# ishine/tts-max

Measured on AMD Instinct MI355X. Metric: audio-codes/sec + RTF@24kHz, TTS-1 bs=1/32, at 1/2/4/8 MI355X, higher is better.
Workload: dtype bf16; 1 GPU; tts1 bf16 bs=1/GPU: prompt 202 tokens (150 codes), 500 greedy codes, codec codec-24k on 650 codes; model=TTS-1 (Llama-3.2-1B dims, V=193856, tied) + xcodec2-style codec codec-24k, global_batch=1, seq_len=702, parallelism=dp1

## Files before the change

### tts-max_amd/csrc/lm_attn_core.h

```cpp
#pragma once
#include "hip_common.h"

namespace tts {

template <int D, int PW>
struct DecShape {
  static constexpr int MT = PW / 16;
  static constexpr int KS = D / 32;
  static constexpr int PS = PW / 32;
  static constexpr int DT = D / 16;
};

constexpr int DEC_G = 4;
constexpr int DEC_NW = 16;
template <int D> constexpr int dec_nw() { return 16; }
template <int D> constexpr int dec_pw() { return D == 64 ? 64 : 32; }

TTS_DEV int vt_off(int S, int d, int p) {
  return (((d >> 4) * (S >> 5) + (p >> 5)) * 16 + (d & 15)) * 32 + (p & 31);
}

TTS_DEV int dec_pos(int base, int mt, int row) {
  return base + 32 * (mt >> 1) + 8 * (row >> 2) + 4 * (mt & 1) + (row & 3);
}

template <int D, int PW, bool O32 = false>
TTS_DEV void dec_load_k(const bf16_t* kc, int base, int ctx, int lane,
                        u32x4_t (&kf)[DecShape<D, PW>::MT][DecShape<D, PW>::KS]) {
  using C = DecShape<D, PW>;
  const int c = lane & 15, g = lane >> 4;
#pragma unroll
  for (int mt = 0; mt < C::MT; ++mt) {
    const int p = min(dec_pos(base, mt, c), ctx - 1);
#pragma unroll
    for (int ks = 0; ks < C::KS; ++ks)
      kf[mt][ks] = O32 ? *(const u32x4_t*)(kc + (p * D + 32 * ks + 8 * g))
                       : *(const u32x4_t*)(kc + (size_t)p * D + 32 * ks + 8 * g);
  }
}
template <int D, int PW, bool O32 = false>
TTS_DEV void dec_load_v(const bf16_t* vtc, int S, int base, int lane,
                        u32x4_t (&vf)[DecShape<D, PW>::PS][DecShape<D, PW>::DT]) {
  using C = DecShape<D, PW>;
  const int c = lane & 15, g = lane >> 4;
#pragma unroll
  for (int ps = 0; ps < C::PS; ++ps) {
    const int pb = min((base >> 5) + ps, (S >> 5) - 1);
    const int o0 = (pb * 16 + c) * 32 + 8 * g;
#pragma unroll
    for (int dt = 0; dt < C::DT; ++dt)
      vf[ps][dt] = O32 ? *(const u32x4_t*)(vtc + (o0 + dt * 16 * S)) : *(const u32x4_t*)(vtc + o0 + (size_t)dt * 16 * S);
  }
}

TTS_DEV uint32_t bits_sel(uint32_t mask, uint32_t a, uint32_t b) { return (a & mask) | (b & ~mask); }
template <int PW>
TTS_DEV bool dec_tail(int base, int ctx) { return __builtin_amdgcn_readfirstlane(base + PW > ctx - 1) != 0; }
template <int D, int PW>
TTS_DEV void dec_patch_k(int base, int ctx, int lane, const bf16_t* knew,
                         u32x4_t (&kf)[DecShape<D, PW>::MT][DecShape<D, PW>::KS]) {
  using C = DecShape<D, PW>;
  const int c = lane & 15, g = lane >> 4, pn = ctx - 1;
  uint32_t m[C::MT];
#pragma unroll
  for (int mt = 0; mt < C::MT; ++mt) m[mt] = dec_pos(base, mt, c) == pn ? 0xffffffffu : 0u;
#pragma unroll
  for (int ks = 0; ks < C::KS; ++ks) {
    const u32x4_t kn = *(const u32x4_t*)(knew + 32 * ks + 8 * g);
#pragma unroll
    for (int mt = 0; mt < C::MT; ++mt)
#pragma unroll
      for (int q = 0; q < 4; ++q) kf[mt][ks][q] = bits_sel(m[mt], kn[q], kf[mt][ks][q]);
  }
}
template <int D, int PW>
TTS_DEV void dec_patch_v(int base, int ctx, int lane, const bf16_t* vnew,
                         u32x4_t (&vf)[DecShape<D, PW>::PS][DecShape<D, PW>::DT]) {
  using C = DecShape<D, PW>;
  const int c = lane & 15, g = lane >> 4, pn = ctx - 1;
  uint32_t vn[C::DT];
#pragma unroll
  for (int dt = 0; dt < C::DT; ++dt) vn[dt] = vnew[16 * dt + c];
#pragma unroll
  for (int ps = 0; ps < C::PS; ++ps) {
    const int p0 = base + 32 * ps + 8 * g;
    uint32_t keep[4], put[4];
#pragma unroll
    for (int e2 = 0; e2 < 4; ++e2) {
      const int pl = p0 + 2 * e2, ph = pl + 1;
      keep[e2] = (pl < pn ? 0x0000ffffu : 0u) | (ph < pn ? 0xffff0000u : 0u);
      put[e2] = (pl == pn ? 0x0000ffffu : 0u) | (ph == pn ? 0xffff0000u : 0u);
    }
#pragma unroll
    for (int dt = 0; dt < C::DT; ++dt) {
      const uint32_t nv = vn[dt] | (vn[dt] << 16);
#pragma unroll
      for (int e2 = 0; e2 < 4; ++e2) vf[ps][dt][e2] = (vf[ps][dt][e2] & keep[e2]) | (nv & put[e2]);
    }
  }
}

template <int D>
TTS_DEV bf16x8_t dec_qfrag(const bf16_t* qs, int lane, int ks) {
  const int h = (lane & 15) & 3, g = lane >> 4;
  return __builtin_bit_cast(bf16x8_t, *(const u32x4_t*)(qs + h * D + 32 * ks + 8 * g));
}

template <int D, int PW>
TTS_DEV void dec_scores(const u32x4_t (&kf)[DecShape<D, PW>::MT][DecShape<D, PW>::KS], const bf16_t* qs,
                        int base, int ctx, float scale, int lane, bool tail, f32x4_t (&s)[DecShape<D, PW>::MT]) {
  using C = DecShape<D, PW>;
  const int g = lane >> 4;
#pragma unroll
  for (int mt = 0; mt < C::MT; ++mt) s[mt] = f32x4_t{0.f, 0.f, 0.f, 0.f};
#pragma unroll
  for (int ks = 0; ks < C::KS; ++ks) {
    const bf16x8_t qb = dec_qfrag<D>(qs, lane, ks);
#pragma unroll
    for (int mt = 0; mt < C::MT; ++mt)
      s[mt] = __builtin_amdgcn_mfma_f32_16x16x32_bf16(__builtin_bit_cast(bf16x8_t, kf[mt][ks]), qb, s[mt], 0, 0, 0);
  }
#pragma unroll
  for (int mt = 0; mt < C::MT; ++mt)
#pragma unroll
    for (int r = 0; r < 4; ++r) s[mt][r] *= scale;
  __builtin_amdgcn_sched_barrier(0);
  if (tail) {
#pragma unroll
    for (int mt = 0; mt < C::MT; ++mt)
#pragma unroll
      for (int r = 0; r < 4; ++r) s[mt][r] = (dec_pos(base, mt, 4 * g + r) < ctx) ? s[mt][r] : -INFINITY;
    __builtin_amdgcn_sched_barrier(0);
  }
  __builtin_amdgcn_sched_barrier(0);
}

template <int D, int PW>
TTS_DEV void dec_pv(float M, float& lsum, f32x4_t (&s)[DecShape<D, PW>::MT],
                    const u32x4_t (&vf)[DecShape<D, PW>::PS][DecShape<D, PW>::DT], f32x4_t (&o)[DecShape<D, PW>::DT]) {
  using C = DecShape<D, PW>;
#pragma unroll
  for (int mt = 0; mt < C::MT; ++mt)
#pragma unroll
    for (int r = 0; r < 4; ++r) {
      const float p = __builtin_amdgcn_exp2f((s[mt][r] - M) * 1.44269504088896341f);
      lsum += p;
      s[mt][r] = p;
    }
#pragma unroll
  for (int ps = 0; ps < C::PS; ++ps) {
    const u32x4_t pw = {pack_bf2(s[2 * ps][0], s[2 * ps][1]), pack_bf2(s[2 * ps][2], s[2 * ps][3]),
                        pack_bf2(s[2 * ps + 1][0], s[2 * ps + 1][1]), pack_bf2(s[2 * ps + 1][2], s[2 * ps + 1][3])};
    const bf16x8_t pb = __builtin_bit_cast(bf16x8_t, pw);
#pragma unroll
    for (int dt = 0; dt < C::DT; ++dt)
      o[dt] = __builtin_amdgcn_mfma_f32_16x16x32_bf16(__builtin_bit_cast(bf16x8_t, vf[ps][dt]), pb, o[dt], 0, 0, 0);
  }
}

template <int D, int NW>
constexpr int dec_red_floats() { return NW * DEC_G * 2 + NW * DEC_G * D; }

template <int D, int PW, int NW, class Bar, bool O32 = false>
TTS_DEV void dec_attend_w(const bf16_t* kc, const bf16_t* vtc, int S, int ctx, float scale, const bf16_t* qs,
                          const bf16_t* knew, const bf16_t* vnew, float* red,
                          u32x4_t (&kf0)[DecShape<D, PW>::MT][DecShape<D, PW>::KS],
                          u32x4_t (&vf0)[DecShape<D, PW>::PS][DecShape<D, PW>::DT], bf16_t* out, int wave,
                          int tid, Bar bar, unsigned long long* stp = nullptr, uint64_t* gout = nullptr,
                          uint32_t gtag = 0) {
  using C = DecShape<D, PW>;
  const int lane = tid & 63;
  const int c = lane & 15, g = lane >> 4;
  const int npass = (ctx + NW * PW - 1) / (NW * PW);
  float* mred = red;
  float* lred = red + NW * DEC_G;
  float* ored = lred + NW * DEC_G;
  const int base0 = wave * PW;

  f32x4_t s0[C::MT];
  float mx = -INFINITY;
  const bool tail0 = dec_tail<PW>(base0, ctx);
  if (base0 < ctx) {
    __builtin_amdgcn_sched_barrier(0);
    if (tail0) {
      dec_patch_k<D, PW>(base0, ctx, lane, knew, kf0);
      __builtin_amdgcn_sched_barrier(0);
    }
    __builtin_amdgcn_sched_barrier(0);
    dec_scores<D, PW>(kf0, qs, base0, ctx, scale, lane, tail0, s0);
#pragma unroll
    for (int mt = 0; mt < C::MT; ++mt)
#pragma unroll
      for (int r = 0; r < 4; ++r) mx = fmaxf(mx, s0[mt][r]);
  }
  for (int ps = 1; ps < npass; ++ps) {
    const int base = (ps * NW + wave) * PW;
    if (base >= ctx) break;
    u32x4_t kf[C::MT][C::KS];
    dec_load_k<D, PW, O32>(kc, base, ctx, lane, kf);
    const bool tail = dec_tail<PW>(base, ctx);
    __builtin_amdgcn_sched_barrier(0);
    if (tail) {
      dec_patch_k<D, PW>(base, ctx, lane, knew, kf);
      __builtin_amdgcn_sched_barrier(0);
    }
    __builtin_amdgcn_sched_barrier(0);
    f32x4_t s[C::MT];
    dec_scores<D, PW>(kf, qs, base, ctx, scale, lane, tail, s);
#pragma unroll
    for (int mt = 0; mt < C::MT; ++mt)
#pragma unroll
      for (int r = 0; r < 4; ++r) mx = fmaxf(mx, s[mt][r]);
  }
  mx = fmaxf(mx, __shfl_xor(mx, 16, 64));
  mx = fmaxf(mx, __shfl_xor(mx, 32, 64));
  if (lane < DEC_G) mred[wave * DEC_G + lane] = mx;
  __builtin_amdgcn_sched_barrier(0);
  if (base0 < ctx && tail0) {
    dec_patch_v<D, PW>(base0, ctx, lane, vnew, vf0);
    __builtin_amdgcn_sched_barrier(0);
  }
  __builtin_amdgcn_sched_barrier(0);
  bar();
  TTS_STAMP(stp, 5);
  float M = -INFINITY;
#pragma unroll
  for (int w = 0; w < NW; ++w) M = fmaxf(M, mred[w * DEC_G + (c & 3)]);

  float lsum = 0.f;
  f32x4_t o[C::DT];
#pragma unroll
  for (int dt = 0; dt < C::DT; ++dt) o[dt] = f32x4_t{0.f, 0.f, 0.f, 0.f};
  if (base0 < ctx) dec_pv<D, PW>(M, lsum, s0, vf0, o);
  for (int ps = 1; ps < npass; ++ps) {
    const int base = (ps * NW + wave) * PW;
    if (base >= ctx) break;
    u32x4_t kf[C::MT][C::KS], vf[C::PS][C::DT];
    dec_load_v<D, PW, O32>(vtc, S, base, lane, vf);
    dec_load_k<D, PW, O32>(kc, base, ctx, lane, kf);
    const bool tail = dec_tail<PW>(base, ctx);
    __builtin_amdgcn_sched_barrier(0);
    if (tail) {
      dec_patch_k<D, PW>(base, ctx, lane, knew, kf);
      __builtin_amdgcn_sched_barrier(0);
    }
    __builtin_amdgcn_sched_barrier(0);
    f32x4_t s[C::MT];
    dec_scores<D, PW>(kf, qs, base, ctx, scale, lane, tail, s);
    if (tail) {
      dec_patch_v<D, PW>(base, ctx, lane, vnew, vf);
      __builtin_amdgcn_sched_barrier(0);
    }
    __builtin_amdgcn_sched_barrier(0);
    dec_pv<D, PW>(M, lsum, s, vf, o);
  }
  lsum += __shfl_xor(lsum, 16, 64);
  lsum += __shfl_xor(lsum, 32, 64);
  if (c < DEC_G) {
#pragma unroll
    for (int dt = 0; dt < C::DT; ++dt)
      *(float4*)(ored + (wave * DEC_G + c) * D + 16 * dt + 4 * g) = make_float4(o[dt][0], o[dt][1], o[dt][2], o[dt][3]);
    if (g == 0) lred[wave * DEC_G + c] = lsum;
  }
  bar();
  TTS_STAMP(stp, 6);
  static_assert(DEC_G * D <= NW * 64, "one output element per thread");
  bf16_t gob = 0;
  for (int i = tid; i < DEC_G * D; i += NW * 64) {
    const int h = i / D, d = i - h * D;
    float v[NW];
#pragma unroll
    for (int w = 0; w < NW; ++w) v[w] = lred[w * DEC_G + h];
    float O = 0.f, L = 0.f;
#pragma unroll
    for (int w = 0; w < NW; ++w) L += v[w];
#pragma unroll
    for (int w = 0; w < NW; ++w) v[w] = ored[(w * DEC_G + h) * D + d];
#pragma unroll
    for (int w = 0; w < NW; ++w) O += v[w];
    const bf16_t ob = f2bf(O / L);
    out[h * D + d] = ob;
    if (gout) gob = ob;
  }
  if (gout) {
    const uint32_t nb = (uint32_t)__builtin_amdgcn_update_dpp(0, (int)gob, 0xB1, 0xf, 0xf, false);
    if (tid < DEC_G * D && !(tid & 1))
      __hip_atomic_store(gout + (tid >> 1), ((uint64_t)gtag << 32) | (nb << 16) | gob, __ATOMIC_RELAXED,
                         __HIP_MEMORY_SCOPE_AGENT);
  }
}

template <int D, int PW, int NW, bool O32 = false>
TTS_DEV void dec_attend(const bf16_t* kc, const bf16_t* vtc, int S, int ctx, float scale, const bf16_t* qs,
                        const bf16_t* knew, const bf16_t* vnew, float* red,
                        u32x4_t (&kf0)[DecShape<D, PW>::MT][DecShape<D, PW>::KS],
                        u32x4_t (&vf0)[DecShape<D, PW>::PS][DecShape<D, PW>::DT], bf16_t* out,
                        unsigned long long* stp = nullptr, uint64_t* gout = nullptr, uint32_t gtag = 0) {
  auto bar = [] { lds_barrier(); };
  dec_attend_w<D, PW, NW, decltype(bar), O32>(kc, vtc, S, ctx, scale, qs, knew, vnew, red, kf0, vf0, out,
                          __builtin_amdgcn_readfirstlane(threadIdx.x >> 6), threadIdx.x, bar, stp, gout, gtag);
}

TTS_DEV float rope_elem(bf16_t x, bf16_t xr, bool lower_half, float c, float sn) {
  const float rot = lower_half ? -bf2f(xr) : bf2f(xr);
  return rbf(rbf(bf2f(x) * c) + rbf(rot * sn));
}

}
```

### tts-max_amd/csrc/lm_gemm_kernel.h

```cpp
#pragma once
#include <algorithm>
#include <cstdio>
#include <stdexcept>
#include <type_traits>

#include "hip_common.h"
#include "lm_kernels.h"
#include "lm_attn_core.h"

namespace tts {

constexpr int wgemm_ea(int waves) { return waves >= 16 ? 1 : (waves >= 8 ? 2 : 4); }
__host__ __device__ inline int wgemm_red_floats(int waves, int ksplit, int ng, int mt, int M, int Kl) {
  const int upw = waves / ksplit;
  int r = upw * (ksplit - 1) * ng * mt * 4 * 64;
  r = r > upw * mt * 16 * 2 ? r : upw * mt * 16 * 2;
  const int segs = (M * (Kl / 8) + 63) / 64;
  r = r > segs ? r : segs;
  r = r > Kl / 2 ? r : Kl / 2;
  return r + 64;
}

constexpr int wgemm_fattn_d(int ku) { return ku == 2 ? 64 : 128; }
template <int D>
constexpr size_t fattn_lds_bytes() {
  return (size_t)(DEC_G * D + 2 * D) * 2 + (size_t)dec_red_floats<D, DEC_NW>() * 4;
}
template <typename Poll>
TTS_DEV bool fattn_wait(Poll ready, int* err, int spins, bool report) {
  for (int n = 1; !ready(); ++n) {
    if (n > spins) {
      if (report) __hip_atomic_store(err, 1, __ATOMIC_RELAXED, __HIP_MEMORY_SCOPE_AGENT);
      return false;
    }
    if ((n & 511) == 0 && __hip_atomic_load(err, __ATOMIC_RELAXED, __HIP_MEMORY_SCOPE_AGENT)) return false;
    __builtin_amdgcn_s_sleep(1);
  }
  return true;
}

template <int NT, int D>
TTS_DEV void fattn_consumer(const WgemmArgs& wa, char* smem, int b) {
  static_assert(NT == DEC_NW * 64, "the fused attention runs on 16-wave workgroups");
  constexpr int PW = dec_pw<D>(), G = DEC_G, H2 = D / 2;
  using C = DecShape<D, PW>;
  const AttnArgs& a = wa.fa;
  bf16_t* qs = (bf16_t*)smem;
  bf16_t* knew = qs + G * D;
  bf16_t* vnew = knew + D;
  float* red = (float*)(vnew + D);
  const int tid = threadIdx.x, lane = tid & 63;
  const int wave = __builtin_amdgcn_readfirstlane(tid >> 6);
  const int row = b / a.KVH, kvh = b % a.KVH;
  const int slot = a.row_slot[row], pos = a.row_pos[row], ctx = pos + 1;
  const size_t kvbase = ((size_t)slot * a.KVH + kvh) * a.max_seq * D;
  const bf16_t* kc = a.kcache + kvbase;
  const bf16_t* vtc = a.vtcache + kvbase;
  unsigned long long* stp = wa.stamps ? wa.stamps + (size_t)blockIdx.x * 32 : nullptr;
  TTS_STAMP(stp, 0);
  u32x4_t kf[C::MT][C::KS], vf[C::PS][C::DT];
  if (wave * PW < ctx) {
    dec_load_k<D, PW, D == 128>(kc, wave * PW, ctx, lane, kf);
    dec_load_v<D, PW, D == 128>(vtc, a.max_seq, wave * PW, lane, vf);
  }
  const int qd = (2 * tid) % D;
  const uint32_t cs2 = *(const uint32_t*)(a.rope_cos + (size_t)pos * D + qd);
  const uint32_t sn2 = *(const uint32_t*)(a.rope_sin + (size_t)pos * D + qd);

  const uint32_t tag = ((uint32_t)pos << 6) | (uint32_t)wa.fattn_layer;
  const int nq = G * D / 2, ngr = nq + D;
  uint32_t raw = 0;
  if (tid < ngr) {
    int col;
    if (tid < nq) col = kvh * G * D + 2 * tid;
    else if (tid < nq + D / 2) col = a.H * D + kvh * D + 2 * (tid - nq);
    else col = a.H * D + a.KVH * D + kvh * D + 2 * (tid - nq - D / 2);
    const uint64_t* gp = wa.gran + (size_t)row * (a.ld_qkv / 2) + col / 2;
    uint64_t v;
    fattn_wait([&] {
      v = __hip_atomic_load(gp, __ATOMIC_RELAXED, __HIP_MEMORY_SCOPE_AGENT);
      return (uint32_t)(v >> 32) == tag;
    }, wa.fattn_err, wa.fattn_spins, true);
    raw = (uint32_t)v;
  }
#ifdef TTS_STAMPS
  lds_barrier();
#endif
  TTS_STAMP(stp, 1);
  const uint32_t rawr = (uint32_t)__shfl_xor((int)raw, D / 4, 64);
  if (tid < ngr) {
    uint32_t w = raw;
    if (tid < nq + D / 2) {
      const bool lower = qd < H2;
      w = pack_bf2(rope_elem((bf16_t)raw, (bf16_t)rawr, lower, bf_lo(cs2), bf_lo(sn2)),
                   rope_elem((bf16_t)(raw >> 16), (bf16_t)(rawr >> 16), lower, bf_hi(cs2), bf_hi(sn2)));
    }
    ((uint32_t*)qs)[tid] = w;
  }
  lds_barrier();
  TTS_STAMP(stp, 2);
  dec_attend<D, PW, DEC_NW, D == 128>(kc, vtc, a.max_seq, ctx, a.scale, qs, knew, vnew, red, kf, vf,
                            a.out + (size_t)row * a.H * D + kvh * G * D, stp,
                            wa.fo_units ? wa.gran + (size_t)wa.M * (wa.N / 2) + (size_t)row * (a.H * D / 2) + kvh * G * D / 2
                                        : nullptr,
                            tag);
  TTS_STAMP(stp, 3);
  if (tid < D) {
    a.kcache[kvbase + (size_t)pos * D + tid] = knew[tid];
    a.vtcache[kvbase + vt_off(a.max_seq, tid, pos)] = vnew[tid];
  }
}

TTS_DEV bf16x8_t as_bf16x8(u32x4_t v) { return __builtin_bit_cast(bf16x8_t, v); }

template <int KU, int KSPLIT, int R>
TTS_DEV void fused_oproj(const WgemmArgs& a, bf16_t* xs, float* red, int wave, int lane, uint32_t tag, int u) {
  const int kpart = wave % KSPLIT;
  const int nr = min(a.fo_ur, a.fo_units);
  u32x4_t wr[R][KU];
#pragma unroll
  for (int st = 0; st < R; ++st)
#pragma unroll
    for (int kk = 0; kk < KU; ++kk)
      wr[st][kk] = __builtin_nontemporal_load((const u32x4_t*)a.fo_w +
                                              ((((long long)st * nr + u) * KSPLIT + kpart) * KU + kk) * 64 + lane);
  const bf16_t rr = a.fo_resid[u * 16 + (lane & 15)];
  const uint64_t* g = a.gran + a.N / 2 + kpart * 64 + lane;
  uint64_t v;
  fattn_wait([&] {
    v = __hip_atomic_load(g, __ATOMIC_RELAXED, __HIP_MEMORY_SCOPE_AGENT);
    return (bool)__all((uint32_t)(v >> 32) == tag);
  }, a.fattn_err, a.fattn_spins, lane == 0);
  *(uint32_t*)(xs + kpart * 128 + 2 * lane) = (uint32_t)v;
  asm volatile("s_waitcnt lgkmcnt(0)" ::: "memory");
  f32x4_t acc = {0.f, 0.f, 0.f, 0.f};
  const int akoff = 8 * (lane >> 4);
#pragma unroll
  for (int st = 0; st < R; ++st)
#pragma unroll
    for (int kk = 0; kk < KU; ++kk) {
      const int k = ((kpart * R + st) * KU + kk) * 32 + akoff;
      const u32x4_t av = *(const u32x4_t*)(xs + k);
      acc = __builtin_amdgcn_mfma_f32_16x16x32_bf16(as_bf16x8(av), as_bf16x8(wr[st][kk]), acc, 0, 0, 0);
    }
  if (kpart > 0) *(f32x4_t*)(red + ((size_t)(kpart - 1) * 64 + lane) * 4) = acc;
  lds_barrier();
  if (kpart == 0) {
    constexpr int HB = 8;
#pragma unroll
    for (int p0 = 1; p0 < KSPLIT; p0 += HB) {
      f32x4_t pv[HB];
#pragma unroll
      for (int j = 0; j < HB; ++j)
        if (p0 + j < KSPLIT) pv[j] = *(const f32x4_t*)(red + ((size_t)(p0 + j - 1) * 64 + lane) * 4);
#pragma unroll
      for (int j = 0; j < HB; ++j)
        if (p0 + j < KSPLIT) acc += pv[j];
    }
    if (lane < 16) a.fo_resid[u * 16 + lane] = f2bf(bf2f(rr) + rbf(acc[0]));
  }
}

template <int KU, int KSPLIT, int R>
TTS_DEV void fused_oproj_rows(const WgemmArgs& a, bf16_t* xs, float* red, int wave, int lane, int u) {
  const int M = a.M, HD = a.fa.H * a.fa.D, ldxs = HD + 8, hid = a.fo_units * 16;
  unsigned long long* stp = a.stamps ? a.stamps + (size_t)blockIdx.x * 32 : nullptr;
  TTS_STAMP(stp, 0);
  const int kpart = wave % KSPLIT;
  const int nr = min(a.fo_ur, a.fo_units);
  const int KTc = (HD >> 5) / a.fo_kc, kt_pc = KTc / KSPLIT, Sc = kt_pc / KU;
  auto ktile = [&](int st, int kk) {
    const int ch = st / Sc;
    return ch * KTc + kpart * kt_pc + (st - ch * Sc) * KU + kk;
  };
  u32x4_t wr[R][KU];
#pragma unroll
  for (int st = 0; st < R; ++st)
#pragma unroll
    for (int kk = 0; kk < KU; ++kk)
      wr[st][kk] = __builtin_nontemporal_load((const u32x4_t*)a.fo_w +
                                              ((((long long)st * nr + u) * KSPLIT + kpart) * KU + kk) * 64 + lane);
  bf16_t rr[4];
#pragma unroll
  for (int r = 0; r < 4; ++r) rr[r] = a.fo_resid[(size_t)min(4 * (lane >> 4) + r, M - 1) * hid + u * 16 + (lane & 15)];
  constexpr int NGL = R * KU >= 4 ? R * KU / 4 : 1;
  int col[NGL];
#pragma unroll
  for (int j = 0; j < NGL; ++j) {
    const int gi = j * 64 + lane, ktl = gi >> 4;
    col[j] = ktile(ktl / KU, ktl % KU) * 32 + (gi & 15) * 2;
  }
  const uint64_t* g0 = a.gran + (size_t)M * (a.N / 2);
  constexpr int RB = NGL >= 4 ? 1 : 4;
  for (int m0 = 0; m0 < M; m0 += RB) {
    uint32_t tag[RB];
#pragma unroll
    for (int rb = 0; rb < RB; ++rb)
      tag[rb] = ((uint32_t)a.fa.row_pos[min(m0 + rb, M - 1)] << 6) | (uint32_t)a.fattn_layer;
    uint64_t v[RB][NGL];
    fattn_wait([&] {
      bool ok = true;
#pragma unroll
      for (int rb = 0; rb < RB; ++rb)
#pragma unroll
        for (int j = 0; j < NGL; ++j) {
          v[rb][j] = __hip_atomic_load(g0 + (size_t)min(m0 + rb, M - 1) * (HD / 2) + col[j] / 2, __ATOMIC_RELAXED,
                                       __HIP_MEMORY_SCOPE_AGENT);
          ok = ok && (uint32_t)(v[rb][j] >> 32) == tag[rb];
        }
      return (bool)__all(ok);
    }, a.fattn_err, a.fattn_spins, lane == 0);
#pragma unroll
    for (int rb = 0; rb < RB; ++rb)
      if (m0 + rb < M) {
#pragma unroll
        for (int j = 0; j < NGL; ++j) *(uint32_t*)(xs + (size_t)(m0 + rb) * ldxs + col[j]) = (uint32_t)v[rb][j];
      }
    if (m0 == 0) TTS_STAMP(stp, 1);
  }
  TTS_STAMP(stp, 2);
  asm volatile("s_waitcnt lgkmcnt(0)" ::: "memory");
  f32x4_t acc = {0.f, 0.f, 0.f, 0.f};
  const bf16_t* xr = xs + (size_t)min(lane & 15, M - 1) * ldxs + 8 * (lane >> 4);
#pragma unroll
  for (int st = 0; st < R; ++st)
#pragma unroll
    for (int kk = 0; kk < KU; ++kk) {
      const u32x4_t av = *(const u32x4_t*)(xr + ktile(st, kk) * 32);
      acc = __builtin_amdgcn_mfma_f32_16x16x32_bf16(as_bf16x8(av), as_bf16x8(wr[st][kk]), acc, 0, 0, 0);
    }
  if (kpart > 0) *(f32x4_t*)(red + ((size_t)(kpart - 1) * 64 + lane) * 4) = acc;
  lds_barrier();
  if (kpart == 0) {
    constexpr int HB = 8;
#pragma unroll
    for (int p0 = 1; p0 < KSPLIT; p0 += HB) {
      f32x4_t pv[HB];
#pragma unroll
      for (int j = 0; j < HB; ++j)
        if (p0 + j < KSPLIT) pv[j] = *(const f32x4_t*)(red + ((size_t)(p0 + j - 1) * 64 + lane) * 4);
#pragma unroll
      for (int j = 0; j < HB; ++j)
        if (p0 + j < KSPLIT) acc += pv[j];
    }
#pragma unroll
    for (int r = 0; r < 4; ++r) {
      const int m = 4 * (lane >> 4) + r;
      if (m < M) a.fo_resid[(size_t)m * hid + u * 16 + (lane & 15)] = f2bf(bf2f(rr[r]) + rbf(acc[r]));
    }
  }
  TTS_STAMP(stp, 3);
}


TTS_DEV void argmax_merge(float& v, int& i, float v2, int i2) {
  if (v2 > v || (v2 == v && i2 < i)) { v = v2; i = i2; }
}

constexpr int A_GLOBAL = 0, A_LDS = 1;

template <int WAVES, int KU, int MT_MAX, int NG, int KSPLIT, int ASRC, bool NORM, int EPI, int R,
          bool EARLY, int KSW = KSPLIT, bool FROWS = false>
__global__ __launch_bounds__(WAVES * 64) void wgemm_kernel(WgemmArgs a) {
  extern __shared__ __attribute__((aligned(16))) char smem[];
  constexpr int NT = WAVES * 64;
  constexpr bool FATT = EPI == EPI_STORE && ASRC == A_LDS && WAVES == DEC_NW && KSW == KSPLIT && MT_MAX == 1 &&
                        ((EARLY && !FROWS && wgemm_fattn_d(KU) == 64) || (!EARLY && FROWS));
  const int fo_wgs = (FATT && a.fattn_wgs) ? a.fo_units : 0;
  const int nproj = (int)gridDim.x - (FATT ? a.fattn_wgs : 0) - fo_wgs;
  if constexpr (FATT) {
    if (a.fattn_wgs) {
      const int cb = (int)blockIdx.x - nproj;
      if (cb >= 0 && cb < a.fattn_wgs) {
        fattn_consumer<NT, wgemm_fattn_d(KU)>(a, smem, cb);
        return;
      }
      if (cb >= a.fattn_wgs) {
        const int lane = threadIdx.x & 63;
        const int wave = __builtin_amdgcn_readfirstlane(threadIdx.x >> 6);
        const size_t xs_bytes = (((size_t)a.M * (a.K + 8) * 2 + 15) & ~(size_t)15);
        if constexpr (FROWS) {
          fused_oproj_rows<KU, KSPLIT, R>(a, (bf16_t*)smem, (float*)(smem + xs_bytes), wave, lane, cb - a.fattn_wgs);
        } else {
          const uint32_t tag = ((uint32_t)a.fa.row_pos[0] << 6) | (uint32_t)a.fattn_layer;
          fused_oproj<KU, KSPLIT, R>(a, (bf16_t*)smem, (float*)(smem + xs_bytes), wave, lane, tag, cb - a.fattn_wgs);
        }
        return;
      }
    }
  }
  constexpr int UPW = WAVES / KSW;
  constexpr int SL = KSPLIT / KSW;
  const int bx = (int)blockIdx.x;
  unsigned long long* stp = a.stamps ? a.stamps + (size_t)blockIdx.x * 32 : nullptr;
  TTS_STAMP(stp, 0);
  const int lane = threadIdx.x & 63;
  const int wave = __builtin_amdgcn_readfirstlane(threadIdx.x >> 6);
  const int kq = wave % KSW;
  const int kpart = (SL > 1 ? (int)blockIdx.y * KSW : 0) + kq;
  const int ugrp = wave / KSW;
  const int M = a.M;
  const int mtn = (M + 15) >> 4;
  const int cs2 = a.csplit == 2 ? 1 : 0;
  const int bunits = (a.N >> 4) / NG;
  const int units = bunits << cs2;
  const int kc = a.kc;
  const int KT = a.sliced ? (a.K >> 5) * kc : (a.K >> 5) * SL;
  const int KTc = KT / kc;
  const int kt_pc = KTc / KSPLIT;
  const int Sc = kt_pc / KU;
  const int st_off = a.sliced ? blockIdx.y * Sc : 0;
  const int kt_base = a.sliced ? blockIdx.y * KTc : (SL > 1 ? (int)blockIdx.y * (a.K >> 5) : 0);
  const bf16_t* xg = a.x ? a.x + ((a.sliced || SL > 1) ? (size_t)blockIdx.y * a.K : 0) : nullptr;
  const int ldxs = a.K + 8;
  const int ustride = nproj * UPW;

  bf16_t* xs = (bf16_t*)smem;
  const size_t xs_bytes = (ASRC != A_GLOBAL) ? (((size_t)M * ldxs * 2 + 15) & ~(size_t)15) : 0;
  float* red = (float*)(smem + xs_bytes);

  const int ur = a.ur;
  auto stile = [&](int uu, int st) -> long long {
    uu = min(uu, units - 1) >> cs2;
    const int r = uu / ur, ui = uu - r * ur;
    const int nr = min(ur, bunits - r * ur);
    return (long long)r * ur * KT * NG + (((long long)(st + st_off) * nr + ui) * KSPLIT + kpart) * NG * KU;
  };
  const int S = a.sliced ? Sc : kc * Sc;

  const int tid = threadIdx.x;
  const int kch = a.K >> 3;
  constexpr bool FTAGS = FATT && !EARLY;
  int ftag_pos = 0;
  if constexpr (FTAGS) {
    if (a.fattn_wgs) ftag_pos = a.fa.row_pos[min(lane & 15, M - 1)];
  }
  constexpr int EA = wgemm_ea(WAVES);
  const int achunks = M * kch;
  const int a_nj = (achunks + NT - 1) / NT;
  constexpr bool early_a = EARLY && ASRC == A_LDS;
  u32x4_t xe[EA], ne[EA];
  if constexpr (early_a) {
    {
#pragma unroll
      for (int j = 0; j < EA; ++j) {
        const int c = min(tid + j * NT, achunks - 1);
        const int m = c / kch, k = (c - m * kch) * 8;
        xe[j] = *(const u32x4_t*)(xg + (size_t)m * a.ldx + k);
        if constexpr (NORM) ne[j] = *(const u32x4_t*)(a.normw + k);
      }
    }
  }
  constexpr bool glds_ok = ASRC == A_LDS && !early_a;
  constexpr bool use_glds = glds_ok;
  if constexpr (glds_ok) {
    if (use_glds) {
      const int ppr = a.K >> 9;
      const int pieces = M * ppr;
      for (int p = wave; p < pieces; p += WAVES) {
        const int m = p / ppr, kp = p - m * ppr;
        __builtin_amdgcn_global_load_lds((gptr_t)(xg + (size_t)m * a.ldx + kp * 512 + lane * 8),
                                         (lptr_t)(xs + (size_t)m * ldxs + kp * 512), 16, 0, 0);
      }
      if constexpr (NORM) {
        for (int p = wave; p < ppr; p += WAVES)
          __builtin_amdgcn_global_load_lds((gptr_t)(a.normw + p * 512 + lane * 8), (lptr_t)((bf16_t*)red + p * 512),
                                           16, 0, 0);
      }
    }
  }
  int u = bx * UPW + ugrp;
  const int u_first = min(u, units - 1);
  bf16_t rre[MT_MAX][4];
  int eosr[MT_MAX][4];
  uint32_t seen_cur[MT_MAX][4];
#pragma unroll
  for (int mt = 0; mt < MT_MAX; ++mt)
#pragma unroll
    for (int r = 0; r < 4; ++r) {
      const int m = min(mt * 16 + 4 * (lane >> 4) + r, M - 1);
      if constexpr (EPI == EPI_RESID) {
        rre[mt][r] = a.resid[(size_t)m * a.ldo + (u_first >> cs2) * 16 + (lane & 15)];
      }
      if constexpr (EPI == EPI_LOGITS) {
        eosr[mt][r] = a.eos_mask[m];
        seen_cur[mt][r] = a.seen[(size_t)m * a.seen_stride + (u_first >> 1)];
      }
    }

  uint32_t ftag = 0;
  if constexpr (FATT && EARLY) {
    if (a.fattn_wgs) ftag = ((uint32_t)a.fa.row_pos[0] << 6) | (uint32_t)a.fattn_layer;
  }

  const uint32_t wbytes = (uint32_t)((long long)(a.N >> 4) * KT * 1024);
  const __amdgpu_buffer_rsrc_t wrsrc = __builtin_amdgcn_make_buffer_rsrc((void*)a.w, (short)0, (int)wbytes, 0x00020000);
  constexpr uint32_t kPast = kWgemmSentinel - (uint32_t)(NG * KU - 1) * 1024u;
  auto soff = [&](int uu, int st) -> uint32_t {
    const int ls = cs2 ? ((lane & ~8) | ((min(uu, units - 1) & 1) << 3)) : lane;
    return uu < units ? (uint32_t)stile(uu, st) * 1024u + (uint32_t)ls * 16u : kPast;
  };
  u32x4_t wr[R][KU][NG];
  constexpr bool AGR = ASRC == A_GLOBAL && MT_MAX <= 2;
  const int arow = lane & 15;
  const int akoff = 8 * (lane >> 4);
  u32x4_t ar[R][KU][AGR ? MT_MAX : 1];
  int pu = u, ps = 0;
  auto issue = [&](u32x4_t (&dst)[KU][NG], u32x4_t (&adst)[KU][AGR ? MT_MAX : 1]) {
    const uint32_t q = soff(pu, ps);
#pragma unroll
    for (int kk = 0; kk < KU; ++kk)
#pragma unroll
      for (int g = 0; g < NG; ++g)
        dst[kk][g] = __builtin_amdgcn_raw_buffer_load_b128(wrsrc, (int)(q + (uint32_t)((g * KU + kk) * 1024)), 0, 2);
    if constexpr (AGR) {
      const int sg = ps + st_off, ch = kc == 1 ? 0 : sg / Sc;
      const int kt = ch * KTc + kpart * kt_pc + (sg - ch * Sc) * KU - kt_base;
#pragma unroll
      for (int kk = 0; kk < KU; ++kk)
#pragma unroll
        for (int mt = 0; mt < MT_MAX; ++mt) {
          const int m = min(mt * 16 + arow, M - 1);
          adst[kk][mt] = *(const u32x4_t*)(xg + (size_t)m * a.ldx + (kt + kk) * 32 + akoff);
        }
    }
    if (++ps == S) { ps = 0; pu += ustride; }
  };
  __builtin_amdgcn_sched_barrier(0);
  if (a.diag & kWgemmDiagMask & 8) __syncthreads();
#pragma unroll
  for (int j = 0; j < R; ++j) issue(wr[j], ar[j]);
  __builtin_amdgcn_sched_barrier(0);

  if (a.diag & kWgemmDiagMask & 1) {
  } else if constexpr (ASRC == A_LDS) {
   if constexpr (early_a) {
    if constexpr (NORM) {
#pragma unroll
      for (int j = 0; j < EA; ++j) {
        if (j < a_nj) {
          const float s = wave_sum_dpp(chunk_sumsq(xe[j]));
          const int c = tid + j * NT;
          if (lane == 0 && c < achunks) red[c >> 6] = s;
        }
      }
      lds_barrier();
    }
#pragma unroll
    for (int j = 0; j < EA; ++j) {
      if (j < a_nj) {
        const int c = tid + j * NT;
        if (c < achunks) {
          const int m = c / kch, k = (c - m * kch) * 8;
          u32x4_t v = xe[j];
          if constexpr (NORM) {
            const int seg0 = (m * kch) >> 6, nseg = kch >> 6;
            float ss = 0.f;
            for (int sg = 0; sg < nseg; ++sg) ss += red[seg0 + sg];
            const float r = 1.0f / sqrtf(ss / (float)a.K + a.eps);
#pragma unroll
            for (int q = 0; q < 4; ++q) {
              v[q] = pack_bf2(bf_lo(ne[j][q]) * rbf(bf_lo(v[q]) * r), bf_hi(ne[j][q]) * rbf(bf_hi(v[q]) * r));
            }
// ... 464 lines not shown
```

Baseline: 1738 audio-codes/s.

## Compute new-token score via MFMA, trim attention reduction to active waves

The decode attention no longer patches the new K row into register fragments on the tail tile. It computes the new token's score with a separate small MFMA and splices it into the masked scores, and the V patch uses a uniform relative offset instead of per-element position compares. The cross-wave max and sum reductions now cover only the number of waves that actually hold context, rounded up to a quarter of the waves through compile-time variants, which cuts LDS reads at short contexts. In fused o-proj, only the one useful float per lane is reduced through LDS instead of full f32x4 vectors, and timing stamps are added. The changes add code-path variants and more tail-handling complexity.

```diff
diff --git a/tts-max_amd/csrc/lm_attn_core.h b/tts-max_amd/csrc/lm_attn_core.h
--- a/tts-max_amd/csrc/lm_attn_core.h
+++ b/tts-max_amd/csrc/lm_attn_core.h
@@ -1,4 +1,6 @@
 #pragma once
+#include <type_traits>
+
 #include "hip_common.h"
 
 namespace tts {
@@ -53,43 +55,34 @@
   }
 }
 
-TTS_DEV uint32_t bits_sel(uint32_t mask, uint32_t a, uint32_t b) { return (a & mask) | (b & ~mask); }
 template <int PW>
 TTS_DEV bool dec_tail(int base, int ctx) { return __builtin_amdgcn_readfirstlane(base + PW > ctx - 1) != 0; }
 template <int D, int PW>
-TTS_DEV void dec_patch_k(int base, int ctx, int lane, const bf16_t* knew,
-                         u32x4_t (&kf)[DecShape<D, PW>::MT][DecShape<D, PW>::KS]) {
-  using C = DecShape<D, PW>;
-  const int c = lane & 15, g = lane >> 4, pn = ctx - 1;
-  uint32_t m[C::MT];
-#pragma unroll
-  for (int mt = 0; mt < C::MT; ++mt) m[mt] = dec_pos(base, mt, c) == pn ? 0xffffffffu : 0u;
-#pragma unroll
-  for (int ks = 0; ks < C::KS; ++ks) {
-    const u32x4_t kn = *(const u32x4_t*)(knew + 32 * ks + 8 * g);
-#pragma unroll
-    for (int mt = 0; mt < C::MT; ++mt)
-#pragma unroll
-      for (int q = 0; q < 4; ++q) kf[mt][ks][q] = bits_sel(m[mt], kn[q], kf[mt][ks][q]);
-  }
-}
-template <int D, int PW>
 TTS_DEV void dec_patch_v(int base, int ctx, int lane, const bf16_t* vnew,
                          u32x4_t (&vf)[DecShape<D, PW>::PS][DecShape<D, PW>::DT]) {
   using C = DecShape<D, PW>;
-  const int c = lane & 15, g = lane >> 4, pn = ctx - 1;
+  const int c = lane & 15, g = lane >> 4;
+  const int rel = __builtin_amdgcn_readfirstlane(ctx - 1 - base);
   uint32_t vn[C::DT];
 #pragma unroll
   for (int dt = 0; dt < C::DT; ++dt) vn[dt] = vnew[16 * dt + c];
 #pragma unroll
   for (int ps = 0; ps < C::PS; ++ps) {
-    const int p0 = base + 32 * ps + 8 * g;
+    const int rp = rel - 32 * ps;
+    if (C::PS > 1 && rp >= 32) continue;
+    if (C::PS > 1 && rp < 0) {
+#pragma unroll
+      for (int dt = 0; dt < C::DT; ++dt) vf[ps][dt] = u32x4_t{0u, 0u, 0u, 0u};
+      continue;
+    }
+    const int gs = rp >> 3, es = (rp >> 1) & 3;
+    const uint32_t hk = (rp & 1) ? 0x0000ffffu : 0u, hp = (rp & 1) ? 0xffff0000u : 0x0000ffffu;
     uint32_t keep[4], put[4];
 #pragma unroll
     for (int e2 = 0; e2 < 4; ++e2) {
-      const int pl = p0 + 2 * e2, ph = pl + 1;
-      keep[e2] = (pl < pn ? 0x0000ffffu : 0u) | (ph < pn ? 0xffff0000u : 0u);
-      put[e2] = (pl == pn ? 0x0000ffffu : 0u) | (ph == pn ? 0xffff0000u : 0u);
+      const uint32_t ke = e2 < es ? 0xffffffffu : (e2 == es ? hk : 0u), pe = e2 == es ? hp : 0u;
+      keep[e2] = g < gs ? 0xffffffffu : (g == gs ? ke : 0u);
+      put[e2] = g == gs ? pe : 0u;
     }
 #pragma unroll
     for (int dt = 0; dt < C::DT; ++dt) {
@@ -108,7 +101,8 @@
 
 template <int D, int PW>
 TTS_DEV void dec_scores(const u32x4_t (&kf)[DecShape<D, PW>::MT][DecShape<D, PW>::KS], const bf16_t* qs,
-                        int base, int ctx, float scale, int lane, bool tail, f32x4_t (&s)[DecShape<D, PW>::MT]) {
+                        const bf16_t* knew, int base, int ctx, float scale, int lane, bool tail,
+                        f32x4_t (&s)[DecShape<D, PW>::MT]) {
   using C = DecShape<D, PW>;
   const int g = lane >> 4;
 #pragma unroll
@@ -126,10 +120,32 @@
     for (int r = 0; r < 4; ++r) s[mt][r] *= scale;
   __builtin_amdgcn_sched_barrier(0);
   if (tail) {
-#pragma unroll
-    for (int mt = 0; mt < C::MT; ++mt)
-#pragma unroll
-      for (int r = 0; r < 4; ++r) s[mt][r] = (dec_pos(base, mt, 4 * g + r) < ctx) ? s[mt][r] : -INFINITY;
+    f32x4_t sn = {0.f, 0.f, 0.f, 0.f};
+#pragma unroll
+    for (int ks = 0; ks < C::KS; ++ks) {
+      const bf16x8_t kn = __builtin_bit_cast(bf16x8_t, *(const u32x4_t*)(knew + 32 * ks + 8 * g));
+      sn = __builtin_amdgcn_mfma_f32_16x16x32_bf16(kn, dec_qfrag<D>(qs, lane, ks), sn, 0, 0, 0);
+    }
+    const float snew = sn[0] * scale;
+    const int rel = __builtin_amdgcn_readfirstlane(ctx - 1 - base);
+#pragma unroll
+    for (int ps = 0; ps < C::PS; ++ps) {
+      const int rp = rel - 32 * ps;
+      if (C::PS > 1 && rp >= 32) continue;
+      if (C::PS > 1 && rp < 0) {
+#pragma unroll
+        for (int h = 0; h < 2; ++h) s[2 * ps + h] = f32x4_t{-INFINITY, -INFINITY, -INFINITY, -INFINITY};
+        continue;
+      }
+      const int d = rp - 8 * g;
+#pragma unroll
+      for (int h = 0; h < 2; ++h)
+#pragma unroll
+        for (int r = 0; r < 4; ++r) {
+          const float beyond = 4 * h + r == d ? snew : -INFINITY;
+          s[2 * ps + h][r] = 4 * h + r < d ? s[2 * ps + h][r] : beyond;
+        }
+    }
     __builtin_amdgcn_sched_barrier(0);
   }
   __builtin_amdgcn_sched_barrier(0);
@@ -160,6 +176,20 @@
 
 template <int D, int NW>
 constexpr int dec_red_floats() { return NW * DEC_G * 2 + NW * DEC_G * D; }
+
+template <int NW, int PW>
+TTS_DEV int dec_ladder(int ctx) {
+  static_assert(NW % 4 == 0, "four ladder steps");
+  const int na = (ctx + PW - 1) / PW;
+  return __builtin_amdgcn_readfirstlane(min(NW, (na + NW / 4 - 1) / (NW / 4) * (NW / 4)));
+}
+template <int NW, class F>
+TTS_DEV void dec_ladder_call(int nl, F f) {
+  if (nl <= NW / 4) f(std::integral_constant<int, NW / 4>{});
+  else if (nl <= NW / 2) f(std::integral_constant<int, NW / 2>{});
+  else if (nl <= 3 * NW / 4) f(std::integral_constant<int, 3 * NW / 4>{});
+  else f(std::integral_constant<int, NW>{});
+}
 
 template <int D, int PW, int NW, class Bar, bool O32 = false>
 TTS_DEV void dec_attend_w(const bf16_t* kc, const bf16_t* vtc, int S, int ctx, float scale, const bf16_t* qs,
@@ -176,18 +206,13 @@
   float* lred = red + NW * DEC_G;
   float* ored = lred + NW * DEC_G;
   const int base0 = wave * PW;
+  const int nl = dec_ladder<NW, PW>(ctx);
 
   f32x4_t s0[C::MT];
   float mx = -INFINITY;
   const bool tail0 = dec_tail<PW>(base0, ctx);
   if (base0 < ctx) {
-    __builtin_amdgcn_sched_barrier(0);
-    if (tail0) {
-      dec_patch_k<D, PW>(base0, ctx, lane, knew, kf0);
-      __builtin_amdgcn_sched_barrier(0);
-    }
-    __builtin_amdgcn_sched_barrier(0);
-    dec_scores<D, PW>(kf0, qs, base0, ctx, scale, lane, tail0, s0);
+    dec_scores<D, PW>(kf0, qs, knew, base0, ctx, scale, lane, tail0, s0);
 #pragma unroll
     for (int mt = 0; mt < C::MT; ++mt)
 #pragma unroll
@@ -199,14 +224,8 @@
     u32x4_t kf[C::MT][C::KS];
     dec_load_k<D, PW, O32>(kc, base, ctx, lane, kf);
     const bool tail = dec_tail<PW>(base, ctx);
-    __builtin_amdgcn_sched_barrier(0);
-    if (tail) {
-      dec_patch_k<D, PW>(base, ctx, lane, knew, kf);
-      __builtin_amdgcn_sched_barrier(0);
-    }
-    __builtin_amdgcn_sched_barrier(0);
     f32x4_t s[C::MT];
-    dec_scores<D, PW>(kf, qs, base, ctx, scale, lane, tail, s);
+    dec_scores<D, PW>(kf, qs, knew, base, ctx, scale, lane, tail, s);
 #pragma unroll
     for (int mt = 0; mt < C::MT; ++mt)
 #pragma unroll
@@ -214,7 +233,7 @@
   }
   mx = fmaxf(mx, __shfl_xor(mx, 16, 64));
   mx = fmaxf(mx, __shfl_xor(mx, 32, 64));
-  if (lane < DEC_G) mred[wave * DEC_G + lane] = mx;
+  if (lane < DEC_G && wave < nl) mred[wave * DEC_G + lane] = mx;
   __builtin_amdgcn_sched_barrier(0);
   if (base0 < ctx && tail0) {
     dec_patch_v<D, PW>(base0, ctx, lane, vnew, vf0);
@@ -224,8 +243,12 @@
   bar();
   TTS_STAMP(stp, 5);
   float M = -INFINITY;
-#pragma unroll
-  for (int w = 0; w < NW; ++w) M = fmaxf(M, mred[w * DEC_G + (c & 3)]);
+  if (base0 < ctx) {
+    dec_ladder_call<NW>(nl, [&](auto NL) {
+#pragma unroll
+      for (int w = 0; w < decltype(NL)::value; ++w) M = fmaxf(M, mred[w * DEC_G + (c & 3)]);
+    });
+  }
 
   float lsum = 0.f;
   f32x4_t o[C::DT];
@@ -239,14 +262,8 @@
     dec_load_v<D, PW, O32>(vtc, S, base, lane, vf);
     dec_load_k<D, PW, O32>(kc, base, ctx, lane, kf);
     const bool tail = dec_tail<PW>(base, ctx);
-    __builtin_amdgcn_sched_barrier(0);
-    if (tail) {
-      dec_patch_k<D, PW>(base, ctx, lane, knew, kf);
-      __builtin_amdgcn_sched_barrier(0);
-    }
-    __builtin_amdgcn_sched_barrier(0);
     f32x4_t s[C::MT];
-    dec_scores<D, PW>(kf, qs, base, ctx, scale, lane, tail, s);
+    dec_scores<D, PW>(kf, qs, knew, base, ctx, scale, lane, tail, s);
     if (tail) {
       dec_patch_v<D, PW>(base, ctx, lane, vnew, vf);
       __builtin_amdgcn_sched_barrier(0);
@@ -256,7 +273,7 @@
   }
   lsum += __shfl_xor(lsum, 16, 64);
   lsum += __shfl_xor(lsum, 32, 64);
-  if (c < DEC_G) {
+  if (c < DEC_G && wave < nl) {
 #pragma unroll
     for (int dt = 0; dt < C::DT; ++dt)
       *(float4*)(ored + (wave * DEC_G + c) * D + 16 * dt + 4 * g) = make_float4(o[dt][0], o[dt][1], o[dt][2], o[dt][3]);
@@ -268,16 +285,19 @@
   bf16_t gob = 0;
   for (int i = tid; i < DEC_G * D; i += NW * 64) {
     const int h = i / D, d = i - h * D;
-    float v[NW];
-#pragma unroll
-    for (int w = 0; w < NW; ++w) v[w] = lred[w * DEC_G + h];
     float O = 0.f, L = 0.f;
-#pragma unroll
-    for (int w = 0; w < NW; ++w) L += v[w];
-#pragma unroll
-    for (int w = 0; w < NW; ++w) v[w] = ored[(w * DEC_G + h) * D + d];
-#pragma unroll
-    for (int w = 0; w < NW; ++w) O += v[w];
+    dec_ladder_call<NW>(nl, [&](auto NL) {
+      constexpr int N = decltype(NL)::value;
+      float v[N];
+#pragma unroll
+      for (int w = 0; w < N; ++w) v[w] = lred[w * DEC_G + h];
+#pragma unroll
+      for (int w = 0; w < N; ++w) L += v[w];
+#pragma unroll
+      for (int w = 0; w < N; ++w) v[w] = ored[(w * DEC_G + h) * D + d];
+#pragma unroll
+      for (int w = 0; w < N; ++w) O += v[w];
+    });
     const bf16_t ob = f2bf(O / L);
     out[h * D + d] = ob;
     if (gout) gob = ob;
diff --git a/tts-max_amd/csrc/lm_gemm_kernel.h b/tts-max_amd/csrc/lm_gemm_kernel.h
--- a/tts-max_amd/csrc/lm_gemm_kernel.h
+++ b/tts-max_amd/csrc/lm_gemm_kernel.h
@@ -115,6 +115,8 @@
 
 template <int KU, int KSPLIT, int R>
 TTS_DEV void fused_oproj(const WgemmArgs& a, bf16_t* xs, float* red, int wave, int lane, uint32_t tag, int u) {
+  unsigned long long* stp = a.stamps ? a.stamps + (size_t)blockIdx.x * 32 : nullptr;
+  TTS_STAMP(stp, 0);
   const int kpart = wave % KSPLIT;
   const int nr = min(a.fo_ur, a.fo_units);
   u32x4_t wr[R][KU];
@@ -131,6 +133,7 @@
     v = __hip_atomic_load(g, __ATOMIC_RELAXED, __HIP_MEMORY_SCOPE_AGENT);
     return (bool)__all((uint32_t)(v >> 32) == tag);
   }, a.fattn_err, a.fattn_spins, lane == 0);
+  TTS_STAMP(stp, 1);
   *(uint32_t*)(xs + kpart * 128 + 2 * lane) = (uint32_t)v;
   asm volatile("s_waitcnt lgkmcnt(0)" ::: "memory");
   f32x4_t acc = {0.f, 0.f, 0.f, 0.f};
@@ -143,22 +146,19 @@
       const u32x4_t av = *(const u32x4_t*)(xs + k);
       acc = __builtin_amdgcn_mfma_f32_16x16x32_bf16(as_bf16x8(av), as_bf16x8(wr[st][kk]), acc, 0, 0, 0);
     }
-  if (kpart > 0) *(f32x4_t*)(red + ((size_t)(kpart - 1) * 64 + lane) * 4) = acc;
+  TTS_STAMP(stp, 2);
+  if (kpart > 0 && lane < 16) red[(kpart - 1) * 16 + lane] = acc[0];
   lds_barrier();
   if (kpart == 0) {
-    constexpr int HB = 8;
-#pragma unroll
-    for (int p0 = 1; p0 < KSPLIT; p0 += HB) {
-      f32x4_t pv[HB];
-#pragma unroll
-      for (int j = 0; j < HB; ++j)
-        if (p0 + j < KSPLIT) pv[j] = *(const f32x4_t*)(red + ((size_t)(p0 + j - 1) * 64 + lane) * 4);
-#pragma unroll
-      for (int j = 0; j < HB; ++j)
-        if (p0 + j < KSPLIT) acc += pv[j];
-    }
-    if (lane < 16) a.fo_resid[u * 16 + lane] = f2bf(bf2f(rr) + rbf(acc[0]));
-  }
+    float pv[KSPLIT > 1 ? KSPLIT - 1 : 1];
+#pragma unroll
+    for (int p = 1; p < KSPLIT; ++p) pv[p - 1] = red[(p - 1) * 16 + (lane & 15)];
+    float r0 = acc[0];
+#pragma unroll
+    for (int p = 1; p < KSPLIT; ++p) r0 += pv[p - 1];
+    if (lane < 16) a.fo_resid[u * 16 + lane] = f2bf(bf2f(rr) + rbf(r0));
+  }
+  TTS_STAMP(stp, 3);
 }
 
 template <int KU, int KSPLIT, int R>
```

Result: faster. 1759 audio-codes/s, median of 6 (+1.2%).
